# gyroflow/gyroflow

Measured on NVIDIA H100. Metric: 4K frames/sec (fisheye+RS warp), higher is better.
Workload: dtype f32

## Files before the change

### gyroflow_b200/csrc/c_abi.cu

```cuda
#include <cuda_runtime.h>
#include <cstdio>
#include <cstring>
#include <cstdlib>
#include <mutex>
#include <cmath>
#include <algorithm>
#include <string>
#include <vector>

#include "kernel_registry.h"
#include "c_abi_internal.h"
#include "gyro_dev.h"
#include <nvtx3/nvToolsExt.h>

using namespace gf;

namespace {

struct Slot {
    GrowBuf<float, true> h_mat, h_mesh;
    GrowBuf<float> d_mat, d_mesh;
    GrowBuf<double> d_mesh64;
    Event done;
};
constexpr int kSlots = 4;
constexpr int kPackedBlockY = 4;
constexpr unsigned long long kMaxOutRows = 65535ull * GF_BLOCK_Y;
static_assert(2 * kPackedBlockY == GF_BLOCK_Y, "the packed kernel's row blocks cover GF_BLOCK_Y rows, like the scalar kernels'");

struct LayoutInfo { int bpp, channels, scalar; float max_value; };
constexpr LayoutInfo kLayouts[LAY_COUNT] = {
    { 1, 1, SC_U8,  255.0f },          { 2, 2, SC_U8,  255.0f },          { 3, 3, SC_U8,  255.0f },   { 4, 4, SC_U8,  255.0f },
    { 2, 1, SC_U16, 65535.0f },        { 4, 2, SC_U16, 65535.0f },        { 6, 3, SC_U16, 65535.0f }, { 8, 4, SC_U16, 65535.0f },
    { 4, 1, SC_F32, 3.402823466e38f }, { 16, 4, SC_F32, 3.402823466e38f }, { 8, 4, SC_F16, 3.402823466e38f },
};

struct Combo {
    int lens = 0, digital = 0, layout = 0;
    KernelFn kernels[KV_COUNT] = {};
    bool no_filter = false;
    int bpp() const { return kLayouts[layout].bpp; }
};

}

struct gf_cuda_ctx {
    int device = 0;
    Combo combo;
    int interpolation = 0;
    int width = 0, height = 0, output_width = 0, output_height = 0;
    KernelFn fn_shade = nullptr;
    GrowBuf<uint32_t> const_flags;
    GrowBuf<uint32_t> vflags;
    cudaStream_t last_stream = nullptr;
    Event last_call;
    FilterPrepass filter;
    int overlays = 0;
    GrowBuf<uint8_t, true> h_drawing;
    GrowBuf<uint8_t> d_drawing, src_ovl;
    PlaneStaging plane_staging;
    size_t host_in_len = 0, host_out_len = 0;
    GrowBuf<uint2> coords;
    Stream stream;
    size_t max_rows = 0;
    Slot slots[kSlots];
    int next_slot = 0;
    unsigned long long launches = 0;
    std::string last_error;
};

namespace {

int pix_layout(int pixel_type) {
    static constexpr int kPixLayout[GF_PIX_COUNT] = { LAY_1U8, LAY_1U16, LAY_3U8, LAY_4U8, LAY_4U8, LAY_3U16, LAY_4U16, LAY_4U16,
                                                      LAY_4F32, LAY_4F16, LAY_1F32, LAY_2U8, LAY_2U16 };
    return (pixel_type >= 0 && pixel_type < GF_PIX_COUNT) ? kPixLayout[pixel_type] : -1;
}

KernelFn find_kernel(const Combo& c, int interp, KernelVariant v) {
    switch (c.lens) {
    case GF_LENS_OPENCV_FISHEYE:     return gf_kernel_opencv_fisheye(c.digital, c.layout, interp, v);
    case GF_LENS_OPENCV_STANDARD:    return gf_kernel_opencv_standard(c.digital, c.layout, interp, v);
    case GF_LENS_POLY3:              return gf_kernel_poly3(c.digital, c.layout, interp, v);
    case GF_LENS_POLY5:              return gf_kernel_poly5(c.digital, c.layout, interp, v);
    case GF_LENS_PTLENS:             return gf_kernel_ptlens(c.digital, c.layout, interp, v);
    case GF_LENS_INSTA360:           return gf_kernel_insta360(c.digital, c.layout, interp, v);
    case GF_LENS_SONY:               return gf_kernel_sony(c.digital, c.layout, interp, v);
    case GF_LENS_GENERIC_POLYNOMIAL: return gf_kernel_generic_polynomial(c.digital, c.layout, interp, v);
    case GF_LENS_GOPRO:              return gf_kernel_gopro(c.digital, c.layout, interp, v);
    default: return nullptr;
    }
}

bool make_combo(int pixel_type, int lens, int digital, int interp, Combo* c) {
    c->layout = pix_layout(pixel_type); c->lens = lens; c->digital = digital;
    const bool no_lean = getenv("GF_DISABLE_LEAN") != nullptr;
    const bool no_packed = no_lean || getenv("GF_DISABLE_X2") != nullptr;
    c->no_filter = getenv("GF_DISABLE_FILTER") != nullptr;
    for (int v = 0; v < KV_COUNT; ++v)
        c->kernels[v] = ((no_packed && v >= KV_PACKED) || (no_lean && v == KV_LEAN)) ? nullptr : find_kernel(*c, interp, (KernelVariant)v);
    return c->layout >= 0;
}

const char* const kLensNames[GF_LENS_COUNT] = {
    "none", "opencv_fisheye", "opencv_standard", "poly3", "poly5", "ptlens", "insta360", "sony", "generic_polynomial",
    "gopro", "gopro_superview", "gopro_hyperview", "gopro_warp", "digital_stretch", "gopro6_superview" };

int validate(std::string* err, const gf_kernel_params* p, const gf_buffer_desc* in, const gf_buffer_desc* out, int bpp) {
    if (!p || !in || !out) return fail(err, GF_ERR_BAD_PARAMS, "null argument");
    if (in->height < 4 || out->height < 4 || p->height < 4 || p->output_height < 4)
        return fail(err, GF_ERR_SIZE_TOO_SMALL, "SizeTooSmall: height < 4");
    if (p->stride < 1 || p->output_stride < 1) return fail(err, GF_ERR_BAD_STRIDE, "InvalidStride: stride < 1");
    if (p->width > 16384 || p->output_width > 16384 || p->width < 1 || p->output_width < 1)
        return fail(err, GF_ERR_BAD_PARAMS, "width out of range (1..16384)");
    if (in->width > p->stride)         return fail(err, GF_ERR_BAD_STRIDE, "InvalidStride: input width > stride");
    if (out->width > p->output_stride) return fail(err, GF_ERR_BAD_STRIDE, "InvalidStride: output width > output_stride");
    if (p->stride != in->stride || p->output_stride != out->stride)
        return fail(err, GF_ERR_BAD_STRIDE, "InvalidStride: KernelParams stride differs from the buffer description");
    if (p->bytes_per_pixel != bpp) return fail(err, GF_ERR_BAD_PARAMS, "bytes_per_pixel does not match the pixel type");
    if (p->matrix_count < 1) return fail(err, GF_ERR_BAD_PARAMS, "matrix_count < 1");
    if ((in->kind != GF_BUF_HOST && in->kind != GF_BUF_DEVICE) || (out->kind != GF_BUF_HOST && out->kind != GF_BUF_DEVICE) || !in->ptr || !out->ptr)
        return fail(err, GF_ERR_BAD_PARAMS, "unsupported buffer source");
    const long long x0 = p->source_rect[0], y0 = p->source_rect[1], x1 = x0 + p->source_rect[2], y1 = y0 + p->source_rect[3];
    if (p->source_rect[2] > 0 && p->source_rect[3] > 0) {
        if (x0 < 0 || y0 < 0) return fail(err, GF_ERR_BUFFER_TOO_SMALL, "source_rect has a negative origin");
        const unsigned long long last = (unsigned long long)(y1 - 1) * (unsigned long long)p->stride + (unsigned long long)x1 * (unsigned long long)bpp;
        if (last > in->len) return fail(err, GF_ERR_BUFFER_TOO_SMALL, "Buffer size mismatch input: source_rect exceeds the input buffer");
    }
    if (out->len == 0) return fail(err, GF_ERR_BUFFER_TOO_SMALL, "empty output buffer");
    const unsigned long long out_rows = (out->len + (unsigned long long)p->output_stride - 1) / (unsigned long long)p->output_stride;
    if (p->output_stride < bpp || out_rows > kMaxOutRows)
        return fail(err, GF_ERR_BAD_PARAMS, "output buffer geometry out of range (a pixel per row, at most 524280 rows)");
    return GF_OK;
}

__global__ void widen_mesh_kernel(const float* __restrict__ m, double* __restrict__ o, int n, float width_f, float height_f) {
    const int i = blockIdx.x * blockDim.x + threadIdx.x;
    if (i < n) o[i] = (double)m[i];
    if (i == 0 && n >= 9) make_mesh_aux(m, width_f, height_f, *reinterpret_cast<MeshAux*>(o + GF_MESH_MAX_LEN));
}
__global__ void __launch_bounds__(1024) scan_tables_kernel(const float* __restrict__ m, size_t rows, uint32_t* flags) {
    __shared__ unsigned warp_or[32];
    unsigned f = 0;
    const size_t n = rows * GF_MATRIX_STRIDE;
    for (size_t i = threadIdx.x; i < n; i += blockDim.x) f |= table_entry_verdict((unsigned)(i % GF_MATRIX_STRIDE), m[i]);
    f = __reduce_or_sync(0xffffffffu, f);
    if ((threadIdx.x & 31u) == 0u) warp_or[threadIdx.x >> 5] = f;
    __syncthreads();
    if (threadIdx.x < 32u) {
        f = threadIdx.x < (blockDim.x >> 5) ? warp_or[threadIdx.x] : 0u;
        f = __reduce_or_sync(0xffffffffu, f);
        if (threadIdx.x == 0u) *flags = f;
    }
}

void fill_uniforms(WarpArgs& A, const Combo& c) {
    const gf_kernel_params* p = &A.p;
    const uint8_t* const src = A.src;
    const uint8_t* const dst = A.dst;
    const int bpp = c.bpp();
    A.out_rows = (int)((A.dst_len + (size_t)p->output_stride - 1) / (size_t)p->output_stride);
    A.out_cols = p->output_stride / bpp;
    const int align = (bpp == 1 || bpp == 2 || bpp == 4 || bpp == 8 || bpp == 16) ? bpp : (bpp == 3 ? 1 : 2);
    uint32_t f = 0;
    if (p->matrix_count > 1) f |= F_RS;
    if ((p->flags & 16) == 16) f |= F_HRS;
    A.r_limit_sq = p->r_limit * p->r_limit;
    if (A.r_limit_sq > 0.0f) f |= F_RLIMIT;
    if (p->light_refraction_coefficient != 1.0f && p->light_refraction_coefficient > 0.0f) f |= F_REFRACT;
    if (A.mesh_len > 0) f |= F_MESH;
    if ((p->flags & 2) == 2 && c.digital != GF_LENS_NONE) f |= F_DIGITAL;
    if (p->input_horizontal_stretch > 0.001f && p->input_horizontal_stretch != 1.0f) f |= F_HSTRETCH;
    if (p->input_vertical_stretch   > 0.001f && p->input_vertical_stretch   != 1.0f) f |= F_VSTRETCH;
    if (p->lens_correction_amount < 1.0f) f |= F_LCA;
    if (p->input_rotation != 0.0f) f |= F_INROT;
    if (p->background_mode == 1) f |= F_BG1;
    if (p->background_mode == 2) f |= F_BG2;
    if (p->background_mode == 3) f |= F_BG3;
    if ((p->flags & 1) == 1) f |= F_FIXRANGE;
    if ((p->flags & 4) == 4) f |= F_FILLBG;
    if (lens_noop(c.lens, p->k)) f |= F_LENS_NOOP;
// ... 154 lines not shown
        }
        if (job.tables_on_device) {
            T.table_flags = job.table_flags_dev ? job.table_flags_dev : ctx->const_flags.ptr + 1;
            T.matrices = job.matrices;
            T.mesh = job.mesh_len ? job.mesh : nullptr;
        } else {
            for (size_t i = 0; i < job.n; ++i) table_rows = std::max(table_rows, (size_t)p[i].matrix_count);
            const size_t mat_bytes = table_rows * GF_MATRIX_STRIDE * sizeof(float);
            memcpy(slot->h_mat.ptr, job.matrices, mat_bytes);
            table_flags = gf_table_flags_host(slot->h_mat.ptr, table_rows);
            CK(err, cudaMemcpyAsync(slot->d_mat.ptr, slot->h_mat.ptr, mat_bytes, cudaMemcpyHostToDevice, st));
            T.matrices = slot->d_mat.ptr;
            if (job.mesh_len) {
                memcpy(slot->h_mesh.ptr, job.mesh, job.mesh_len * sizeof(float));
                CK(err, cudaMemcpyAsync(slot->d_mesh.ptr, slot->h_mesh.ptr, job.mesh_len * sizeof(float), cudaMemcpyHostToDevice, st));
                T.mesh = slot->d_mesh.ptr;
            }
        }
        T.mesh_len = (int)job.mesh_len;
        if (job.mesh_len) {
            double* const m64 = slot->d_mesh64.ptr;
            widen_mesh_kernel<<<(unsigned)((job.mesh_len + 255) / 256), 256, 0, st>>>(T.mesh, m64, (int)job.mesh_len, (float)p->width, (float)p->height);
            CK(err, cudaGetLastError());
            T.mesh64 = m64; T.mesh_aux = reinterpret_cast<const MeshAux*>(m64 + GF_MESH_MAX_LEN);
        }
        if (host) {
            nvtxRangePushA("gf_h2d_frame");
            const int rc = ctx->plane_staging.upload(job.n, job.in, job.out, p, false, st, err, in.data(), out.data());
            nvtxRangePop();
            if (rc != GF_OK) return rc;
            src_private = job.in[0].kind == GF_BUF_HOST;
        }
        return GF_OK;
    }

    int draw_input_overlays() {
        if (!overlays || job.n != 1) return GF_OK;
        bool any_input_stage = false;
        if ((p->flags & GF_FLAG_DRAWING_ENABLED) && job.drawing && job.drawing_len) {
            CK(err, ctx->h_drawing.reserve(job.drawing_len, st));
            CK(err, ctx->d_drawing.reserve(job.drawing_len, st));
            CK(err, cudaStreamSynchronize(st));
            for (size_t i = 0; i < job.drawing_len; ++i) { const uint8_t d = job.drawing[i]; ctx->h_drawing.ptr[i] = d; any_input_stage |= (d != 0 && (d & 1u) == 0u); }
            CK(err, cudaMemcpyAsync(ctx->d_drawing.ptr, ctx->h_drawing.ptr, job.drawing_len, cudaMemcpyHostToDevice, st));
            drawing_dev = ctx->d_drawing.ptr;
        }
        if (!any_input_stage) return GF_OK;
        if (!src_private) {
            CK(err, ctx->src_ovl.reserve(in[0].len, st));
            CK(err, cudaMemcpyAsync(ctx->src_ovl.ptr, in[0].ptr, in[0].len, cudaMemcpyDeviceToDevice, st));
            in[0].ptr = ctx->src_ovl.ptr;
        }
        const LayoutInfo& L = kLayouts[ctx->combo.layout];
        if (gf_internal_draw_overlays((void*)st, (uint8_t*)in[0].ptr, in[0].len, in[0].width, in[0].height, p->stride, p, L.channels, L.scalar, 1,
                                      drawing_dev, job.drawing_len) != GF_OK) return fail(err, GF_ERR_CUDA, "overlay kernel (input stage) failed");
        return GF_OK;
    }

    int render() {
        if (fused) return render_planes(0, job.n);
        for (size_t i = 0; i < job.n; ++i) { const int rc = render_planes(i, 1); if (rc != GF_OK) return rc; }
        return GF_OK;
    }

    int render_planes(size_t first, size_t count) {
        WarpArgs A = T;
        A.p = p[first];
        A.src = (const uint8_t*)in[first].ptr; A.dst = (uint8_t*)out[first].ptr; A.src_len = in[first].len; A.dst_len = out[first].len;
        const uint32_t flags = (size_t)A.p.matrix_count < table_rows ? gf_table_flags_host(slot->h_mat.ptr, (size_t)A.p.matrix_count) : table_flags;
        if (!job.tables_on_device) A.table_flags = ctx->const_flags.ptr + (flags ? 1 : 0);
        fill_uniforms(A, ctx->combo);
        const dim3 grid((A.out_cols + GF_BLOCK_X - 1) / GF_BLOCK_X, (A.out_rows + GF_BLOCK_Y - 1) / GF_BLOCK_Y);
        const Plan plan = plan_frame(ctx->combo, A, flags, job.tables_on_device, count, job.coord_only);
        const FilterPrepass::Table* radial = nullptr;
        if (plan.filter) { const int rc = ctx->filter.table(A.p.k, st, err, &radial); if (rc != GF_OK) return rc; }
        if (plan.two_pass) {
            if (!ctx->fn_shade && !job.coord_only) return fail(err, GF_ERR_UNSUPPORTED_COMBO, "no sampling kernel for this pixel layout");
            CK(err, ctx->coords.reserve((size_t)A.out_cols * (size_t)A.out_rows * (size_t)plan.n_maps, st));
            A.coord_out = ctx->coords.ptr;
        }
        const KernelFn fn = ctx->combo.kernels[plan.kernel];
        if (plan.kernel == KV_PACKED || plan.kernel == KV_PACKED_COORDS) {
            const dim3 block2(GF_BLOCK_X, kPackedBlockY), grid2(grid.x, (A.out_rows + 2 * kPackedBlockY - 1) / (2 * kPackedBlockY));
            if (radial) { const int rc = ctx->filter.launch(fn, grid2, block2, A, *radial, st, err, ctx->launches); if (rc != GF_OK) return rc; }
            else CK(err, launch_pdl(fn, grid2, block2, A, st));
        } else {
            const size_t map_len = (size_t)A.out_cols * (size_t)A.out_rows;
            for (int mi = 0; mi < plan.n_maps; ++mi) {
                if (plan.two_pass) { A.coord_out = ctx->coords.ptr + (size_t)mi * map_len; A.coord_shift = mi; }
                fn<<<grid, kBlock, 0, st>>>(A);
                CK(err, cudaGetLastError());
                if (mi > 0) ctx->launches++;
            }
        }
        CK(err, cudaGetLastError());
        ctx->launches++;
        if (!plan.two_pass || job.coord_only) return GF_OK;
        for (size_t i = first; i < first + count; ++i) {
            WarpArgs B = A;
            B.p = p[i];
            B.coord_out = nullptr; B.coord_in = ctx->coords.ptr; B.coord_maps = plan.n_maps; B.coord_shift = 0;
            B.src = (const uint8_t*)in[i].ptr; B.dst = (uint8_t*)out[i].ptr; B.src_len = in[i].len; B.dst_len = out[i].len;
            fill_uniforms(B, ctx->combo);
            ctx->fn_shade<<<grid, kBlock, 0, st>>>(B);
            CK(err, cudaGetLastError());
            ctx->launches++;
        }
        return GF_OK;
    }

    int finish() {
        if (slot) CK(err, cudaEventRecord(slot->done.get(), st));
        for (size_t i = 0; overlays && i < job.n; ++i) {
            const LayoutInfo& L = kLayouts[ctx->combo.layout];
            if (gf_internal_draw_overlays((void*)st, (uint8_t*)out[i].ptr, out[i].len, out[i].width, out[i].height, p[i].output_stride, &p[i], L.channels,
                                          L.scalar, 0, drawing_dev, job.drawing_len) != GF_OK) return fail(err, GF_ERR_CUDA, "overlay kernel (output stage) failed");
        }
        if (!host) return GF_OK;
        nvtxRangePushA("gf_d2h_frame");
        const int rc = ctx->plane_staging.download(job.n, job.out, p, st, err);
        nvtxRangePop();
        if (rc != GF_OK) return rc;
        if (job.sync_host) CK(err, cudaStreamSynchronize(st));
        return GF_OK;
    }
};

int order_after_last_call(gf_cuda_ctx* ctx, cudaStream_t st) {
    if (ctx->last_stream && ctx->last_stream != st) CK(&ctx->last_error, cudaStreamWaitEvent(st, ctx->last_call.get(), 0));
    ctx->last_stream = st;
    return GF_OK;
}

int check_frame(gf_cuda_ctx* ctx, const FrameJob& job) {
    std::string* const err = &ctx->last_error;
    for (size_t i = 0; i < job.n; ++i) {
        if (job.kind >= 0 && (job.in[i].kind != job.kind || job.out[i].kind != job.kind)) return fail(err, GF_ERR_BAD_PARAMS, job.kind_error);
        const int rc = validate(err, job.p + i, job.in + i, job.out + i, ctx->combo.bpp());
        if (rc != GF_OK) return rc;
    }
    for (size_t i = 0; i < job.n; ++i) {
        const gf_kernel_params* p = &job.p[i];
        if (!job.matrices) return fail(err, GF_ERR_NO_DATA, "NoStabilizationData: matrices is null");
        if (p->width != ctx->width || p->height != ctx->height || p->output_width != ctx->output_width || p->output_height != ctx->output_height)
            return fail(err, GF_ERR_SIZE_MISMATCH, "SizeMismatch: KernelParams size differs from the size this context was created for");
        if (p->interpolation != ctx->interpolation)
            return fail(err, GF_ERR_UNSUPPORTED_COMBO, "interpolation differs from the one this context was created for");
        if ((size_t)p->matrix_count > job.matrix_rows) return fail(err, GF_ERR_BUFFER_TOO_SMALL, "Buffer size mismatch matrices: matrix_count > rows supplied");
        if (!job.tables_on_device && job.matrix_rows > ctx->max_rows) return fail(err, GF_ERR_BUFFER_TOO_SMALL, "Buffer size mismatch matrices");
        if (job.mesh_len > GF_MESH_MAX_LEN) return fail(err, GF_ERR_BUFFER_TOO_SMALL, "Buffer size mismatch buf_mesh_data");
        if (job.mesh_len > 0 && !job.mesh) return fail(err, GF_ERR_BAD_PARAMS, "mesh is null");
        if (job.mesh_len > 0 && job.mesh_len < 9) return fail(err, GF_ERR_BAD_PARAMS, "mesh shorter than its 9-value header (the reference would index out of bounds)");
        if (!job.grow_staging && job.in[i].kind == GF_BUF_HOST && job.in[i].len > ctx->host_in_len)
            return fail(err, GF_ERR_BUFFER_TOO_SMALL, "Buffer size mismatch input");
        if (!job.grow_staging && job.out[i].kind == GF_BUF_HOST && job.out[i].len > ctx->host_out_len)
            return fail(err, GF_ERR_BUFFER_TOO_SMALL, "Buffer size mismatch output");
        if (job.tables_on_device && (reinterpret_cast<uintptr_t>(job.matrices) & 7u)) return fail(err, GF_ERR_BAD_PARAMS, "device matrices must be 8-byte aligned");
    }
    return GF_OK;
}

int run_frame(gf_cuda_ctx* ctx, const FrameJob& job) {
    if (!ctx) return fail(nullptr, GF_ERR_BAD_PARAMS, "ctx is null");
    std::string* const err = &ctx->last_error;
    int rc = check_frame(ctx, job);
    if (rc != GF_OK) return rc;
    CK(err, cudaSetDevice(ctx->device));
// ... 461 lines not shown
```

### gyroflow_b200/csrc/c_abi_internal.h

```cpp
#pragma once
#include <cuda_runtime.h>
#include <cstddef>
#include <cstdint>
#include <memory>
#include <string>
#include <vector>
#include "../../include/gyroflow_cuda.h"
#include "frame_geometry.cuh"

namespace gf {


inline thread_local std::string g_last_error;

inline int fail(std::string* sink, int code, const std::string& msg) {
    g_last_error = msg;
    if (sink) *sink = msg;
    return code;
}
inline int cuda_error(cudaError_t e, const char* what, std::string* sink) {
    (void)cudaGetLastError();
    return fail(sink, GF_ERR_CUDA, std::string(what) + ": " + cudaGetErrorName(e) + " (" + cudaGetErrorString(e) + ")");
}
#define CK(sink, call) do { const cudaError_t e_ = (call); if (e_ != cudaSuccess) return gf::cuda_error(e_, #call, sink); } while (0)


template <class T, bool PINNED = false> struct GrowBuf {
    T* ptr = nullptr; size_t len = 0;
    GrowBuf() = default;
    GrowBuf(GrowBuf&& o) noexcept : ptr(o.ptr), len(o.len) { o.ptr = nullptr; o.len = 0; }
    ~GrowBuf() { release(); }
    cudaError_t reserve(size_t n, cudaStream_t st) {
        if (n <= len) return cudaSuccess;
        if (ptr) { const cudaError_t e = cudaStreamSynchronize(st); if (e != cudaSuccess) return e; release(); }
        const cudaError_t e = PINNED ? cudaMallocHost((void**)&ptr, n * sizeof(T)) : cudaMalloc((void**)&ptr, n * sizeof(T));
        if (e == cudaSuccess) len = n; else ptr = nullptr;
        return e;
    }
private:
    void release() { if (ptr) { if (PINNED) cudaFreeHost(ptr); else cudaFree(ptr); } ptr = nullptr; len = 0; }
};

template <auto Destroy> struct Deleter { template <class T> void operator()(T* h) const { Destroy(h); } };
using Stream = std::unique_ptr<CUstream_st, Deleter<cudaStreamDestroy>>;
using Event = std::unique_ptr<CUevent_st, Deleter<cudaEventDestroy>>;
inline cudaError_t create_stream(Stream& s) {
    cudaStream_t h = nullptr;
    const cudaError_t e = cudaStreamCreateWithFlags(&h, cudaStreamNonBlocking);
    if (e == cudaSuccess) s.reset(h);
    return e;
}
inline cudaError_t create_event(Event& ev) {
    cudaEvent_t h = nullptr;
    const cudaError_t e = cudaEventCreateWithFlags(&h, cudaEventDisableTiming);
    if (e == cudaSuccess) ev.reset(h);
    return e;
}

enum : uint32_t { TBL_WILD = 1u, TBL_IBIS = 2u };
__host__ __device__ __forceinline__ bool tame(float v) { const float a = fabsf(v); return v == 0.0f || (a >= 0x1p-40f && a <= 0x1p40f); }
__host__ __device__ __forceinline__ uint32_t table_entry_verdict(unsigned col, float v) {
    return col < 9u ? (tame(v) ? 0u : TBL_WILD) : (v == 0.0f ? 0u : TBL_IBIS);
}
__host__ __device__ __forceinline__ uint32_t table_row_verdict(const float* r) {
    uint32_t f = 0;
    for (unsigned i = 0; i < GF_MATRIX_STRIDE; ++i) f |= table_entry_verdict(i, r[i]);
    return f;
}

double keyframed(const gf_compute_params* cp, int typ, double timestamp_ms, double dflt);
double fov_unscaled(const gf_compute_params* cp, size_t frame, bool use_fovs, double timestamp_ms, bool for_ui);
void get_new_k(const gf_compute_params* cp, const double* camera_matrix, double fov, double (&new_k)[9]);
struct FrameTiming {
    double frame_readout_time;
    double row_readout_time, start_ts;
    Quat q0;
};
FrameTiming frame_timing(const gf_compute_params* cp, size_t frame, double timestamp_ms, bool can_invert);
CameraStab camera_stab_at(const gf_compute_params* cp, size_t frame, bool framebuffer_inverted, const StabSplines* splines);
bool lens_noop(int lens, const float* k);
bool point_path_supported(int lens, int digital);

struct WarpArgs;
typedef void (*KernelFn)(const WarpArgs);
cudaError_t launch_pdl(KernelFn fn, dim3 g, dim3 b, const WarpArgs& args, cudaStream_t st);
float radial_table_cap(const float* k, float4* rows);
class FilterPrepass {
public:
    struct Table {
        uint32_t key[4] = {};
        float a_cap = 0.0f;
        unsigned long long last_use = 0;
        GrowBuf<float4, true> h; GrowBuf<float4> d; Event done;
    };
    cudaError_t init(int device) { return cudaDeviceGetAttribute(&sm_count, cudaDevAttrMultiProcessorCount, device); }
    int table(const float* k, cudaStream_t st, std::string* err, const Table** out);
    int launch(KernelFn fn, dim3 grid, dim3 block, WarpArgs& A, const Table& t, cudaStream_t st, std::string* err, unsigned long long& launches);
    int stats(cudaStream_t st, std::string* err, uint64_t* out6) const;
private:
    Table tables[4];
    GrowBuf<uint32_t> queue; GrowBuf<unsigned> counts;
    unsigned long long frames = 0, uses = 0, builds = 0;
    int sm_count = 1;
};

bool warp_covers_output(const gf_kernel_params& p, const gf_buffer_desc& out, int bpp);
class PlaneStaging {
public:
    cudaError_t reserve(size_t n, const gf_buffer_desc* in, const gf_buffer_desc* out, cudaStream_t st);
    int check(size_t n, const gf_buffer_desc* in, const gf_buffer_desc* out, std::string* err) const;
    int upload(size_t n, const gf_buffer_desc* in, const gf_buffer_desc* out, const gf_kernel_params* p, bool checksum, cudaStream_t st,
               std::string* err, gf_buffer_desc* din, gf_buffer_desc* dout);
    int download(size_t n, const gf_buffer_desc* out, const gf_kernel_params* p, cudaStream_t st, std::string* err) const;
private:
    std::vector<GrowBuf<uint8_t>> in_, out_;
};

inline gf_compute_params stmap_params(const gf_compute_params& user, int per_frame) {
    gf_compute_params cp = user;
    if (!per_frame) cp.frame_readout_time = 0.0;
    cp.suppress_rotation = 1; cp.fovs = nullptr; cp.n_fovs = 0; cp.minimal_fovs = nullptr; cp.n_minimal_fovs = 0;
    cp.fov_scale = 1.0; cp.output_width = cp.width; cp.output_height = cp.height;
    return cp;
}
inline bool stmap_size_ok(int w, int h) { return w >= 4 && h >= 4 && w <= 32768 && h <= 32768; }

}

int gf_internal_draw_overlays(void* cu_stream, uint8_t* buf_dev, size_t len, int width, int height, int stride, const gf_kernel_params* p,
                              int count, int scalar, int is_input, const uint8_t* drawing_dev, size_t drawing_len);
```

### gyroflow_b200/csrc/filter_prepass.cu

```cuda
#include <cstring>
#include <cmath>
#include <algorithm>
#include "warp_kernel.cuh"
#include "c_abi_internal.h"

using namespace gf;
namespace {

constexpr unsigned kDeferCap = 1u << 20;
constexpr unsigned kTailThreadsPerSM = 2048;

float filter_a_cap(const float* k) {
    auto B = [&](double t) { const double t2 = t * t; return t2 * (fabs((double)k[0]) + t2 * (fabs((double)k[1]) + t2 * (fabs((double)k[2]) + t2 * fabs((double)k[3])))); };
    for (int i = 0; i < 4; ++i) if (!std::isfinite(k[i])) return 0.0f;
    double lo = 0.0, hi = 1.55;
    if (B(hi) > 0.25) { for (int it = 0; it < 60; ++it) { const double mid = 0.5 * (lo + hi); if (B(mid) <= 0.25) lo = mid; else hi = mid; } }
    else lo = hi;
    if (lo < 0.5) return 0.0f;
    const double a = tan(lo) * tan(lo);
    return (float)std::min(a * 0.999, 16000.0);
}

double radial_T(double a) { const double r = sqrt(a); return r < 1e-4 ? 1.0 - a / 3.0 + a * a / 5.0 : atan(r) / r; }
struct RadialGrid {
    static constexpr int N = GF_RADIAL_FIT_ROWS, kChk = 65;
    double lo[N], hi[N], h[N];
    double node_a[N][4], node_T[N][4];
    double chk_a[N][kChk], chk_T[N][kChk];
    double vinv[4][4];
    RadialGrid() {
        double t[4], V[4][8];
        for (int q = 0; q < 4; ++q) t[q] = cos((2 * q + 1) * 3.14159265358979323846 / 8.0);
        for (int r = 0; r < 4; ++r) for (int c = 0; c < 8; ++c) V[r][c] = c < 4 ? pow(1.0 + t[r], c) : (c - 4 == r ? 1.0 : 0.0);
        for (int c = 0; c < 4; ++c) {
            int p = c;
            for (int r = c + 1; r < 4; ++r) if (fabs(V[r][c]) > fabs(V[p][c])) p = r;
            for (int j = 0; j < 8; ++j) std::swap(V[c][j], V[p][j]);
            const double d = V[c][c];
            for (int j = 0; j < 8; ++j) V[c][j] /= d;
            for (int r = 0; r < 4; ++r) if (r != c) { const double f = V[r][c]; for (int j = 0; j < 8; ++j) V[r][j] -= f * V[c][j]; }
        }
        for (int r = 0; r < 4; ++r) for (int c = 0; c < 4; ++c) vinv[r][c] = V[r][c + 4];
        for (int i = 0; i < N; ++i) {
            const int e = i / 16, j = i % 16;
            lo[i] = ldexp(1.0 + j / 16.0, e - 30); hi[i] = ldexp(1.0 + (j + 1) / 16.0, e - 30);
            h[i] = 0.5 * (hi[i] - lo[i]);
            for (int q = 0; q < 4; ++q) { node_a[i][q] = lo[i] + h[i] * (1.0 + t[q]); node_T[i][q] = radial_T(node_a[i][q]); }
            for (int q = 0; q < kChk; ++q) { chk_a[i][q] = (double)(float)(lo[i] + (hi[i] - lo[i]) * q / 64.0); chk_T[i][q] = radial_T(chk_a[i][q]); }
        }
    }
};

float build_radial_table(const float* k, float a_cap, float4* rows) {
    static const RadialGrid* const G = new RadialGrid();
    constexpr double kRadialBudget = 0x1p-23;
    uint32_t cap_bits; memcpy(&cap_bits, &a_cap, 4);
    const int n_valid = std::max(0, std::min(GF_RADIAL_FIT_ROWS, (int)(cap_bits >> 19) - GF_RADIAL_FIT));
    const double k0 = k[0], k1 = k[1], k2 = k[2], k3 = k[3];
    auto R = [&](double a, double T) { const double q = a * T * T; return T * (1.0 + q * (k0 + q * (k1 + q * (k2 + q * k3)))); };
    bool ok = n_valid > 0;
    for (int i = 0; i < GF_RADIAL_ROWS; ++i) rows[i] = make_float4(NAN, NAN, NAN, NAN);
    for (int i = 0; i < n_valid; ++i) {
        double f[4], c[4];
        for (int q = 0; q < 4; ++q) f[q] = R(G->node_a[i][q], G->node_T[i][q]);
        for (int r = 0; r < 4; ++r) c[r] = G->vinv[r][0] * f[0] + G->vinv[r][1] * f[1] + G->vinv[r][2] * f[2] + G->vinv[r][3] * f[3];
        const double hh = G->h[i];
        const float4 row = make_float4((float)c[0], (float)(c[1] / hh), (float)(c[2] / (hh * hh)), (float)(c[3] / (hh * hh * hh)));
        rows[GF_RADIAL_FIT + i] = row;
        for (int q = 0; q < RadialGrid::kChk; ++q) {
            const double a = G->chk_a[i][q], d = a - G->lo[i];
            const double v = row.x + d * (row.y + d * (row.z + d * (double)row.w));
            const double want = R(a, G->chk_T[i][q]);
            if (!(fabs(v - want) <= kRadialBudget * fabs(want))) ok = false;
        }
    }
    for (int i = 0; i < GF_RADIAL_FIT; ++i) rows[i] = rows[GF_RADIAL_FIT];
    uint32_t r_bits = cap_bits & 0xfff80000u; float a_cap_r; memcpy(&a_cap_r, &r_bits, 4);
    return ok ? a_cap_r : 0.0f;
}

}

float gf::radial_table_cap(const float* k, float4* rows) { return build_radial_table(k, filter_a_cap(k), rows); }

int FilterPrepass::table(const float* k, cudaStream_t st, std::string* err, const Table** out) {
    uint32_t key[4]; memcpy(key, k, sizeof(key));
    Table *t = nullptr, *lru = &tables[0];
    for (Table& e : tables) {
        if (e.last_use && memcmp(e.key, key, sizeof(key)) == 0) t = &e;
        if (e.last_use < lru->last_use) lru = &e;
    }
    if (!t) {
        t = lru; t->last_use = 0;
        if (!t->done) CK(err, create_event(t->done));
        CK(err, cudaEventSynchronize(t->done.get()));
        CK(err, t->h.reserve(GF_RADIAL_ROWS, st)); CK(err, t->d.reserve(GF_RADIAL_ROWS, st));
        t->a_cap = radial_table_cap(k, t->h.ptr); builds++;
        CK(err, cudaMemcpyAsync(t->d.ptr, t->h.ptr, GF_RADIAL_ROWS * sizeof(float4), cudaMemcpyHostToDevice, st));
        CK(err, cudaEventRecord(t->done.get(), st));
        memcpy(t->key, key, sizeof(key));
    }
    t->last_use = ++uses;
    *out = t->a_cap > 0.0f ? t : nullptr;
    return GF_OK;
}

int FilterPrepass::launch(KernelFn fn, dim3 grid, dim3 block, WarpArgs& A, const Table& t, cudaStream_t st, std::string* err,
                          unsigned long long& launches) {
    if (!queue.ptr) {
        CK(err, queue.reserve(kDeferCap, st)); CK(err, counts.reserve(2, st));
        CK(err, cudaMemsetAsync(counts.ptr, 0, 2 * sizeof(unsigned), st));
    }
    const unsigned cur = (unsigned)(frames++ & 1ull);
    A.feat |= F_FILTER;
    A.flt.q = queue.ptr; A.flt.cap = (uint32_t)queue.len;
    A.flt.count = counts.ptr + cur; A.flt.count_next = counts.ptr + (cur ^ 1u);
    A.flt.mid_row = A.matrices + (size_t)(A.p.matrix_count / 2) * GF_MATRIX_STRIDE;
    const FilterEps eps = filter_eps(A.p.c[1]);
    A.flt.rtab = t.d.ptr; A.flt.eps_rel = eps.rel; A.flt.eps_abs = eps.abs;
    A.flt.tail = 0;
    CK(err, launch_pdl(fn, grid, block, A, st));
    CK(err, cudaEventRecord(t.done.get(), st));
    A.flt.tail = 1;
    CK(err, launch_pdl(fn, dim3(sm_count * kTailThreadsPerSM / (block.x * block.y)), block, A, st));
    launches++;
    return GF_OK;
}

int FilterPrepass::stats(cudaStream_t st, std::string* err, uint64_t* out6) const {
    unsigned count = 0;
    if (frames > 0) {
        CK(err, cudaMemcpyAsync(&count, counts.ptr + ((frames - 1) & 1ull), sizeof(count), cudaMemcpyDeviceToHost, st));
        CK(err, cudaStreamSynchronize(st));
    }
    out6[0] = frames; out6[1] = count; out6[2] = kDeferCap; out6[3] = (uint64_t)sm_count * kTailThreadsPerSM;
    out6[4] = builds; out6[5] = uses - builds;
    return GF_OK;
}
```

### gyroflow_b200/csrc/warp_kernel.cuh

```cuda
#pragma once
#include "lens_models.cuh"
#include "gf_coeffs_tables.h"
#include "f32x2.cuh"
#include <cuda_fp16.h>

namespace gf {

struct MapC {
    float in_min, mul, div, rcp, add;
    int   fast_div;
    int   identity;
};

__host__ __device__ inline MapC make_map(float in_min, float in_max, float out_min, float out_max, float max_abs_int_coord) {
    MapC m;
    m.in_min = in_min;
    m.mul = out_max - out_min;
    m.div = in_max - in_min;
    m.rcp = 1.0f / m.div;
    m.add = out_min;
    const float ad = fabsf(m.div);
    m.fast_div = (isfinite(m.div) && ad >= 0x1p-40f && ad <= 0x1p40f) ? 1 : 0;
    m.identity = (max_abs_int_coord >= 0.0f && m.mul == m.div && m.mul > 0.0f && in_min == truncf(in_min) &&
                  (max_abs_int_coord + fabsf(in_min)) * m.mul < 16777216.0f) ? 1 : 0;
    return m;
}

enum : uint32_t {
    F_RS         = 1u << 0,
    F_HRS        = 1u << 1,
    F_RLIMIT     = 1u << 2,
    F_REFRACT    = 1u << 3,
    F_MESH       = 1u << 4,
    F_DIGITAL    = 1u << 5,
    F_HSTRETCH   = 1u << 6,
    F_VSTRETCH   = 1u << 7,
    F_LCA        = 1u << 8,
    F_INROT      = 1u << 9,
    F_BG1        = 1u << 10,
    F_BG2        = 1u << 11,
    F_BG3        = 1u << 12,
    F_FIXRANGE   = 1u << 13,
    F_FILLBG     = 1u << 14,
    F_LENS_NOOP  = 1u << 15,
    F_SRC_VEC    = 1u << 16,
    F_DST_VEC    = 1u << 17,
    F_FB_INV     = 1u << 18,
    F_IS_Y       = 1u << 19,
    F_T3D        = 1u << 20,
    F_PIXLIMIT   = 1u << 21,
    F_WILD       = 1u << 22,
    F_INTPRO     = 1u << 23,
    F_FILTER     = 1u << 24,
    F_SRC_VEC8   = 1u << 25,
    F_SHORTROW   = 1u << 26,
};

constexpr uint32_t F_GENERAL_ONLY = F_HRS | F_RLIMIT | F_REFRACT | F_MESH | F_HSTRETCH | F_VSTRETCH | F_LCA | F_INROT |
                                    F_BG1 | F_BG2 | F_BG3 | F_FIXRANGE | F_FILLBG | F_LENS_NOOP | F_FB_INV | F_T3D | F_PIXLIMIT;
constexpr uint32_t F_LEAN_REQUIRED = F_SRC_VEC | F_DST_VEC;

template <bool GEN> __device__ __forceinline__ bool has(uint32_t feat, uint32_t bit) {
    if (GEN) return (feat & bit) != 0;
    if (bit & F_GENERAL_ONLY) return false;
    if (bit & (F_LEAN_REQUIRED | F_DIGITAL)) return true;
    return (feat & bit) != 0;
}

constexpr int GF_RADIAL_ROWS = 8192;
constexpr int GF_RADIAL_FIT = (127 - 30) << 4;
constexpr int GF_RADIAL_FIT_ROWS = (14 + 30) * 16;

constexpr float kFilterRho = 0x1.7p-18f;
struct FilterEps { float rel, abs; };
GF_HD FilterEps filter_eps(float c_y, float rho = kFilterRho) { return { rho + 0x1p-22f, 0x1p-22f * fabsf(c_y) }; }

struct WarpArgs {
    gf_kernel_params p;
    const uint8_t* src;
    uint8_t*       dst;
    const float*   matrices;
    const float*   mesh;
    const double*  mesh64;
    const struct MeshAux* mesh_aux;
    uint2*         coord_out;
    const uint2*   coord_in;
    const uint32_t* table_flags;
    struct X2Filter {
        static constexpr int kMaxCols = 1 << 16, kMaxRows = 2 << 16;
        uint32_t* q;
        unsigned* count;
        unsigned* count_next;
        uint32_t  cap;
        int       tail;
        const float4* rtab;
        const float*  mid_row;
        float     eps_rel, eps_abs;
    } flt;
    int            coord_shift;
    int            coord_maps;
    unsigned long long src_len, dst_len;
    int   mesh_len;
    int   out_rows;
    int   out_cols;
    uint32_t feat;
    float r_limit_sq;
    float out_c[2], out_f[2];
    float bg[4];
    MapC  omap_x, omap_y;
    MapC  smap_x, smap_y;
    float width_f, height_f;
    float frame_w, frame_h;
    float rot_cos, rot_sin;
    int   rs_lim;
    int   row_lim;
    int   u8_limit;
    int   src_rect[4];
    int   interior_span[2];
    struct X2Hot {
        const uint8_t* src;
        int x_off, y_off;
        int x0, x1, y0, y1;
        int full_rows, last_cols;
        int wbias[2];
        unsigned wlim[2];
        int full;
    } hot;
};

enum { SC_U8 = 0, SC_U16 = 1, SC_F32 = 2, SC_F16 = 3 };

template <int COUNT_, int SCALAR_> struct Pix {
    static constexpr int COUNT = COUNT_;
    static constexpr int SCALAR = SCALAR_;
    static constexpr int SBYTES = SCALAR_ == SC_U8 ? 1 : (SCALAR_ == SC_F32 ? 4 : 2);
    static constexpr int BYTES = COUNT_ * SBYTES;
    static constexpr bool POW2 = (BYTES == 1 || BYTES == 2 || BYTES == 4 || BYTES == 8 || BYTES == 16);
    static constexpr int ALIGN = POW2 ? BYTES : SBYTES;

    static GF_DEV float scalar_to_float(uint32_t raw) {
        if (SCALAR == SC_F32) return __uint_as_float(raw);
        if (SCALAR == SC_F16) return __half2float(__ushort_as_half((unsigned short)raw));
        return __uint_as_float(0x4b000000u | raw) - 8388608.0f;
    }
    static GF_DEV uint32_t float_to_scalar(float v) {
        if (SCALAR == SC_F32) return __float_as_uint(v);
        if (SCALAR == SC_F16) {
            const uint32_t b = __float_as_uint(v);
            if (v != v) return ((b >> 16) & 0x8000u) | 0x7e00u | ((b & 0x7fffffu) >> 13);
            return (uint32_t)__half_as_ushort(__float2half_rn(v));
        }
        int i = __float2int_rz(v);
        const int hi = SCALAR == SC_U8 ? 255 : 65535;
        i = i < 0 ? 0 : (i > hi ? hi : i);
        return (uint32_t)i;
    }
    static GF_DEV uint32_t load_scalar(const uint8_t* __restrict__ p) {
        if (SBYTES == 1) return __ldg(p);
        if (SBYTES == 2) return __ldg(reinterpret_cast<const unsigned short*>(p));
        return __ldg(reinterpret_cast<const unsigned int*>(p));
    }
    static GF_DEV void load_raw(const uint8_t* __restrict__ p, uint32_t (&r)[COUNT]) {
        if (!POW2) {
            #pragma unroll
            for (int i = 0; i < COUNT; ++i) r[i] = load_scalar(p + i * SBYTES);
        } else if (BYTES <= 4) {
            const uint32_t w = BYTES == 1 ? (uint32_t)__ldg(p) : (BYTES == 2 ? (uint32_t)__ldg(reinterpret_cast<const unsigned short*>(p)) : __ldg(reinterpret_cast<const unsigned int*>(p)));
            #pragma unroll
            for (int i = 0; i < COUNT; ++i) r[i] = COUNT == 1 ? w : ((w >> (8 * SBYTES * i)) & (SBYTES == 1 ? 0xffu : 0xffffu));
        } else if (BYTES == 8) {
            const uint2 w = __ldg(reinterpret_cast<const uint2*>(p));
            #pragma unroll
// ... 922 lines not shown
```

### gyroflow_b200/csrc/warp_kernel_x2.cuh

```cuda
#pragma once
#include "warp_kernel.cuh"

namespace gf {

using p2::f2;

GF_DEV bool in_window_r2(float a) {
    const uint32_t t = (__float_as_uint(a) << 1) - (71u << 24);
    return t < (104u << 24);
}
GF_DEV bool zero_or_in_window(float v) {
    const uint32_t u = __float_as_uint(v) << 1;
    return u == 0u || (u - (67u << 24)) < (121u << 24);
}

template <int M> struct Lens2 { static constexpr bool kHas = false; };
__host__ __device__ constexpr bool filter_pair(int lens, int digital) { return lens == GF_LENS_OPENCV_FISHEYE && digital == GF_LENS_NONE; }

template <> struct Lens2<GF_LENS_OPENCV_FISHEYE> {
    static constexpr bool kHas = true;
    static GF_DEV bool divisors_ok(float wa, float wb) { return fminf(wa, wb) > 0.0f; }
    static GF_DEV float approx_v(float _x, float _y, float _w, const gf_kernel_params& P, const float4* __restrict__ rtab) {
        const float iw = p2::rcp_approx(_w);
        const float x = _x * iw, y = _y * iw;
// ... 487 lines not shown
template <int LENS, int DIGITAL, class PIX, bool COORD>
static __device__ __noinline__ void finish_pair_cold(const WarpArgs& A, int x, int y0, float pxs, f2 py, uint32_t idx_a, uint32_t idx_b,
                                                     bool wr_a, bool wr_b) {
    const PairUV c = rotate_and_distort_cold<LENS, DIGITAL>(pxs, py.x, py.y, idx_a, idx_b, A, 1);
    const bool ok_a = (c.ok & 1) != 0, ok_b = (c.ok & 2) != 0;
    if (COORD) {
        uint2* const cm_a = A.coord_out + ((size_t)y0 * (size_t)A.out_cols + (size_t)x);
        *cm_a = !wr_a ? make_uint2(GF_COORD_MARK, GF_COORD_SKIP) : (ok_a ? make_uint2(__float_as_uint(c.ua), __float_as_uint(c.va)) : make_uint2(GF_COORD_MARK, GF_COORD_NONE));
        if ((y0 + 1) < A.out_rows) cm_a[A.out_cols] = !wr_b ? make_uint2(GF_COORD_MARK, GF_COORD_SKIP) : (ok_b ? make_uint2(__float_as_uint(c.ub), __float_as_uint(c.vb)) : make_uint2(GF_COORD_MARK, GF_COORD_NONE));
        return;
    }
    const unsigned long long off_a = (unsigned long long)y0 * (unsigned long long)A.p.output_stride + (unsigned long long)x * (unsigned long long)PIX::BYTES;
    int wu_a = 0, wu_b = 0, wv_a = 0, wv_b = 0;
    if (PIX::SCALAR == SC_U8) {
        wu_a = hot_w(c.ua, A.hot.wbias[0]); wv_a = hot_w(c.va, A.hot.wbias[1]);
        wu_b = hot_w(c.ub, A.hot.wbias[0]); wv_b = hot_w(c.vb, A.hot.wbias[1]);
    }
    if (wr_a) shade_lean<PIX>(ok_a, (c.ok & 4) != 0, c.ua, c.va, wu_a, wv_a, A, A.dst + off_a);
    if (wr_b) shade_lean<PIX>(ok_b, (c.ok & 8) != 0, c.ub, c.vb, wu_b, wv_b, A, A.dst + off_a + (unsigned long long)A.p.output_stride);
}

template <int LENS, int DIGITAL, class PIX, bool TRUSTED, bool COORD, bool FULL = false>
GF_DEV void warp_x2_body(const WarpArgs& A, const int x, const int y0, const bool exact_prepass) {
    using namespace p2;
    static_assert(!FULL || DIGITAL == GF_LENS_NONE, "a digital lens may turn a coordinate into -0");
    const gf_kernel_params& P = A.p;
    if (!FULL && (x >= A.out_cols || y0 >= A.out_rows)) return;
    const unsigned long long BYTES = COORD ? (unsigned long long)P.bytes_per_pixel : (unsigned long long)PIX::BYTES;
    const unsigned long long ostride = (unsigned long long)P.output_stride;
    const unsigned long long off_a = (unsigned long long)y0 * ostride + (unsigned long long)x * BYTES;
    const unsigned long long off_b = off_a + ostride;
    float opx, opy_a, opy_b;
    bool wr_a, wr_b;
    if (FULL) {
        wr_a = wr_b = true;
        opx = (float)(x + A.hot.x_off); opy_a = (float)(y0 + A.hot.y_off); opy_b = (float)(y0 + 1 + A.hot.y_off);
    } else if (A.feat & F_INTPRO) {
        const int y1 = y0 + 1;
        const bool in_x = (x >= A.hot.x0) & (x < A.hot.x1);
        wr_a = in_x & (y0 >= A.hot.y0) & (y0 < A.hot.y1);
        wr_b = in_x & (y1 >= A.hot.y0) & (y1 < A.hot.y1);
        if (A.feat & F_SHORTROW) {
            wr_a &= (y0 < A.hot.full_rows) | ((y0 == A.hot.full_rows) & (x < A.hot.last_cols));
            wr_b &= (y1 < A.hot.full_rows) | ((y1 == A.hot.full_rows) & (x < A.hot.last_cols));
        }
        opx = (float)(x + A.hot.x_off); opy_a = (float)(y0 + A.hot.y_off); opy_b = (float)(y1 + A.hot.y_off);
    } else {
        opx = map_apply_int_lean((float)x, A.omap_x);
        opy_a = map_apply_int_lean((float)y0, A.omap_y);
        opy_b = map_apply_int_lean((float)(y0 + 1), A.omap_y);
        const bool in_x = (opx >= 0.0f) & (as_i32(opx) < P.output_width);
        wr_a = in_x & (off_a + BYTES <= A.dst_len) & (opy_a >= 0.0f) & (as_i32(opy_a) < P.output_height);
        wr_b = in_x & ((y0 + 1) < A.out_rows) & (off_b + BYTES <= A.dst_len) & (opy_b >= 0.0f) & (as_i32(opy_b) < P.output_height);
    }
    uint2* const cm_a = COORD ? A.coord_out + ((size_t)y0 * (size_t)A.out_cols + (size_t)x) : nullptr;
    const bool row_b = FULL || (y0 + 1) < A.out_rows;
    if (!FULL && !(wr_a | wr_b)) {
        if (COORD) { *cm_a = make_uint2(GF_COORD_MARK, GF_COORD_SKIP); if (row_b) cm_a[A.out_cols] = make_uint2(GF_COORD_MARK, GF_COORD_SKIP); }
        return;
    }

    const float pxs = opx + P.translation2d[0];
    const f2 px = bc(pxs);
    const f2 py = mk(opy_a + P.translation2d[1], opy_b + P.translation2d[1]);
    const int lim = A.row_lim;
    int sy_a = 0, sy_b = 0;
    do {
        if constexpr (TRUSTED && filter_pair(LENS, DIGITAL)) {
            if (!exact_prepass) {
                const MatRow9 rm = load_row9(A.flt.mid_row, 0u);
                const float bx = pxs * rm.m01.x, by = pxs * rm.m23.y, bw = pxs * rm.m67.x;
                const float xa = (bx + py.x * rm.m01.y) + rm.m23.x, xb = (bx + py.y * rm.m01.y) + rm.m23.x;
                const float ya = (by + py.x * rm.m45.x) + rm.m45.y, yb = (by + py.y * rm.m45.x) + rm.m45.y;
                const float wa = (bw + py.x * rm.m67.y) + rm.m8,    wb = (bw + py.y * rm.m67.y) + rm.m8;
                const float ca = Lens2<LENS>::approx_v(xa, ya, wa, P, A.flt.rtab), cb = Lens2<LENS>::approx_v(xb, yb, wb, P, A.flt.rtab);
                const bool w_ok = Lens2<LENS>::divisors_ok(wa, wb);
                const float ta = ca + P.c[1], tb = cb + P.c[1];
                const float ea = __fmaf_rn(fabsf(ca), A.flt.eps_rel, A.flt.eps_abs), eb = __fmaf_rn(fabsf(cb), A.flt.eps_rel, A.flt.eps_abs);
                const bool ca_ok = certify_row(ta, ea, lim, sy_a), cb_ok = certify_row(tb, eb, lim, sy_b);
                if (w_ok & ca_ok & cb_ok) break;
                const unsigned m = __activemask();
                const unsigned lane = threadIdx.x & 31u;
                const int leader = __ffs((int)m) - 1;
                unsigned base = 0;
                if ((int)lane == leader) base = atomicAdd(A.flt.count, (unsigned)__popc(m));
                base = __shfl_sync(m, base, leader);
                const unsigned slot = base + (unsigned)__popc(m & ((1u << lane) - 1u));
                if (slot < A.flt.cap) { A.flt.q[slot] = (uint32_t)x | ((uint32_t)(y0 >> 1) << 16); return; }
            } else if (!(A.feat & F_RS)) break;
        } else {
            if (!(A.feat & F_RS)) break;
        }
        const uint32_t mid = (uint32_t)P.matrix_count / 2u;
        f2 tu, tv; bool bad = false;
        rotate_and_distort_x2<LENS, DIGITAL, TRUSTED>(px, py, mid, mid, A, tu, tv, bad);
        if (bad) {
            const PairUV c = rotate_and_distort_cold<LENS, DIGITAL>(pxs, py.x, py.y, mid, mid, A, 0);
            tv = mk((c.ok & 1) ? c.va : py.x, (c.ok & 2) ? c.vb : py.y);
        }
        round_away_clamped_x2(tv, lim, sy_a, sy_b);
    } while (false);
    f2 u, v; bool bad = false;
    rotate_and_distort_x2<LENS, DIGITAL, TRUSTED>(px, py, (uint32_t)sy_a, (uint32_t)sy_b, A, u, v, bad);
    u = map_apply_x2<!FULL>(u, A.smap_x, bad);
    v = map_apply_x2<!FULL>(v, A.smap_y, bad);
    if (bad) { finish_pair_cold<LENS, DIGITAL, PIX, COORD>(A, x, y0, pxs, py, (uint32_t)sy_a, (uint32_t)sy_b, wr_a, wr_b); return; }

    if (COORD) {
        *cm_a = !wr_a ? make_uint2(GF_COORD_MARK, GF_COORD_SKIP) : make_uint2(__float_as_uint(u.x), __float_as_uint(v.x));
        if (row_b) cm_a[A.out_cols] = !wr_b ? make_uint2(GF_COORD_MARK, GF_COORD_SKIP) : make_uint2(__float_as_uint(u.y), __float_as_uint(v.y));
        return;
    }
    int wu_a = 0, wu_b = 0, wv_a = 0, wv_b = 0;
    if (PIX::SCALAR == SC_U8) {
        wu_a = hot_w(u.x, A.hot.wbias[0]); wv_a = hot_w(v.x, A.hot.wbias[1]);
        wu_b = hot_w(u.y, A.hot.wbias[0]); wv_b = hot_w(v.y, A.hot.wbias[1]);
        if (wr_a & wr_b & hot_interior(wu_a, wv_a, A) & hot_interior(wu_b, wv_b, A)) {
            constexpr int C = PIX::COUNT;
            uint32_t sa[C], sb[C];
            sample_u8_hot<PIX>(wu_a, wv_a, A, sa);
            sample_u8_hot<PIX>(wu_b, wv_b, A, sb);
            PIX::store_scalars(A.dst + off_a, true, sa);
            PIX::store_scalars(A.dst + off_b, true, sb);
            return;
        }
    }
    if (wr_a) shade_lean<PIX>(true, false, u.x, v.x, wu_a, wv_a, A, A.dst + off_a);
    if (wr_b) shade_lean<PIX>(true, false, u.y, v.y, wu_b, wv_b, A, A.dst + off_b);
}

template <int LENS, int DIGITAL, class PIX, int MINB, bool COORD = false>
__global__ void __launch_bounds__(GF_BLOCK_X * GF_BLOCK_Y, MINB)
warp_kernel_x2(const __grid_constant__ WarpArgs A) {
    constexpr bool kFilter = filter_pair(LENS, DIGITAL);
    asm volatile("griddepcontrol.wait;" ::: "memory");
    const bool trusted = __ldg(A.table_flags) == 0u;
    if constexpr (kFilter) if (A.flt.tail) {
        const unsigned tid = (blockIdx.y * gridDim.x + blockIdx.x) * (blockDim.x * blockDim.y) + threadIdx.y * blockDim.x + threadIdx.x;
        if (tid == 0u) *A.flt.count_next = 0u;
        if (!trusted) return;
        const unsigned n = min(*A.flt.count, A.flt.cap);
        const unsigned stride = gridDim.x * gridDim.y * blockDim.x * blockDim.y;
        for (unsigned i = tid; i < n; i += stride) {
            const uint32_t e = A.flt.q[i];
            warp_x2_body<LENS, DIGITAL, PIX, true, COORD>(A, (int)(e & 0xffffu), (int)(e >> 16) * 2, true);
        }
        return;
    }
    const int x = blockIdx.x * GF_BLOCK_X + threadIdx.x;
    const int y0 = (blockIdx.y * blockDim.y + threadIdx.y) * 2;
    if (trusted) {
        const bool exact_prepass = !(kFilter && (A.feat & F_FILTER));
        if constexpr (DIGITAL == GF_LENS_NONE) if (A.hot.full) { warp_x2_body<LENS, DIGITAL, PIX, true, COORD, true>(A, x, y0, exact_prepass); return; }
        warp_x2_body<LENS, DIGITAL, PIX, true, COORD>(A, x, y0, exact_prepass);
    } else {
        warp_x2_body<LENS, DIGITAL, PIX, false, COORD>(A, x, y0, true);
    }
}

}
```

Before: 11190.

## Shard filter defer-queue counter into padded segments to cut atomic contention

Replaces the single global atomic counter for the deferred-pixel queue with 128 padded per-segment counters and sub-queues, selected by warp row index, so warps enqueueing failed-certification pixels contend less on one address. The tail pass now assigns warps to segments and strides within each segment, and stats sum all segment counts. It also adds an env-controlled epsilon scale for the filter tolerance, which defaults to 1 and so changes nothing by default. The cost is that per-segment capacity is cap/128, so a skewed segment can overflow sooner, and the tail work may be unevenly balanced across segments.

Result: no change. 11240 (median of 6 runs) (+0.5%).

```diff
diff --git a/gyroflow_b200/csrc/c_abi.cu b/gyroflow_b200/csrc/c_abi.cu
--- a/gyroflow_b200/csrc/c_abi.cu
+++ b/gyroflow_b200/csrc/c_abi.cu
@@ -39,6 +39,7 @@
     int lens = 0, digital = 0, layout = 0;
     KernelFn kernels[KV_COUNT] = {};
     bool no_filter = false;
+    float eps_scale = 1.0f;
     int bpp() const { return kLayouts[layout].bpp; }
 };
 
@@ -97,6 +98,7 @@
     const bool no_lean = getenv("GF_DISABLE_LEAN") != nullptr;
     const bool no_packed = no_lean || getenv("GF_DISABLE_X2") != nullptr;
     c->no_filter = getenv("GF_DISABLE_FILTER") != nullptr;
+    if (const char* e = getenv("GF_FILTER_EPS_SCALE")) { const float v = strtof(e, nullptr); if (v >= 1.0f) c->eps_scale = v; }
     for (int v = 0; v < KV_COUNT; ++v)
         c->kernels[v] = ((no_packed && v >= KV_PACKED) || (no_lean && v == KV_LEAN)) ? nullptr : find_kernel(*c, interp, (KernelVariant)v);
     return c->layout >= 0;
@@ -417,7 +419,7 @@
         const KernelFn fn = ctx->combo.kernels[plan.kernel];
         if (plan.kernel == KV_PACKED || plan.kernel == KV_PACKED_COORDS) {
             const dim3 block2(GF_BLOCK_X, kPackedBlockY), grid2(grid.x, (A.out_rows + 2 * kPackedBlockY - 1) / (2 * kPackedBlockY));
-            if (radial) { const int rc = ctx->filter.launch(fn, grid2, block2, A, *radial, st, err, ctx->launches); if (rc != GF_OK) return rc; }
+            if (radial) { const int rc = ctx->filter.launch(fn, grid2, block2, A, *radial, ctx->combo.eps_scale, st, err, ctx->launches); if (rc != GF_OK) return rc; }
             else CK(err, launch_pdl(fn, grid2, block2, A, st));
         } else {
             const size_t map_len = (size_t)A.out_cols * (size_t)A.out_rows;
diff --git a/gyroflow_b200/csrc/c_abi_internal.h b/gyroflow_b200/csrc/c_abi_internal.h
--- a/gyroflow_b200/csrc/c_abi_internal.h
+++ b/gyroflow_b200/csrc/c_abi_internal.h
@@ -95,7 +95,8 @@
     };
     cudaError_t init(int device) { return cudaDeviceGetAttribute(&sm_count, cudaDevAttrMultiProcessorCount, device); }
     int table(const float* k, cudaStream_t st, std::string* err, const Table** out);
-    int launch(KernelFn fn, dim3 grid, dim3 block, WarpArgs& A, const Table& t, cudaStream_t st, std::string* err, unsigned long long& launches);
+    int launch(KernelFn fn, dim3 grid, dim3 block, WarpArgs& A, const Table& t, float eps_scale, cudaStream_t st, std::string* err,
+               unsigned long long& launches);
     int stats(cudaStream_t st, std::string* err, uint64_t* out6) const;
 private:
     Table tables[4];
diff --git a/gyroflow_b200/csrc/filter_prepass.cu b/gyroflow_b200/csrc/filter_prepass.cu
--- a/gyroflow_b200/csrc/filter_prepass.cu
+++ b/gyroflow_b200/csrc/filter_prepass.cu
@@ -1,6 +1,7 @@
 #include <cstring>
 #include <cmath>
 #include <algorithm>
+#include <vector>
 #include "warp_kernel.cuh"
 #include "c_abi_internal.h"
 
@@ -9,6 +10,7 @@
 
 constexpr unsigned kDeferCap = 1u << 20;
 constexpr unsigned kTailThreadsPerSM = 2048;
+constexpr unsigned kCounts = 2 * WarpArgs::X2Filter::kSegs * WarpArgs::X2Filter::kCountStride;
 
 float filter_a_cap(const float* k) {
     auto B = [&](double t) { const double t2 = t * t; return t2 * (fabs((double)k[0]) + t2 * (fabs((double)k[1]) + t2 * (fabs((double)k[2]) + t2 * fabs((double)k[3])))); };
@@ -105,19 +107,19 @@
     return GF_OK;
 }
 
-int FilterPrepass::launch(KernelFn fn, dim3 grid, dim3 block, WarpArgs& A, const Table& t, cudaStream_t st, std::string* err,
-                          unsigned long long& launches) {
+int FilterPrepass::launch(KernelFn fn, dim3 grid, dim3 block, WarpArgs& A, const Table& t, float eps_scale, cudaStream_t st,
+                          std::string* err, unsigned long long& launches) {
     if (!queue.ptr) {
-        CK(err, queue.reserve(kDeferCap, st)); CK(err, counts.reserve(2, st));
-        CK(err, cudaMemsetAsync(counts.ptr, 0, 2 * sizeof(unsigned), st));
+        CK(err, queue.reserve(kDeferCap, st)); CK(err, counts.reserve(kCounts, st));
+        CK(err, cudaMemsetAsync(counts.ptr, 0, kCounts * sizeof(unsigned), st));
     }
     const unsigned cur = (unsigned)(frames++ & 1ull);
     A.feat |= F_FILTER;
-    A.flt.q = queue.ptr; A.flt.cap = (uint32_t)queue.len;
-    A.flt.count = counts.ptr + cur; A.flt.count_next = counts.ptr + (cur ^ 1u);
+    A.flt.q = queue.ptr; A.flt.cap = (uint32_t)(queue.len / WarpArgs::X2Filter::kSegs);
+    A.flt.count = counts.ptr + cur * (kCounts / 2); A.flt.count_next = counts.ptr + (cur ^ 1u) * (kCounts / 2);
     A.flt.mid_row = A.matrices + (size_t)(A.p.matrix_count / 2) * GF_MATRIX_STRIDE;
     const FilterEps eps = filter_eps(A.p.c[1]);
-    A.flt.rtab = t.d.ptr; A.flt.eps_rel = eps.rel; A.flt.eps_abs = eps.abs;
+    A.flt.rtab = t.d.ptr; A.flt.eps_rel = eps.rel * eps_scale; A.flt.eps_abs = eps.abs * eps_scale;
     A.flt.tail = 0;
     CK(err, launch_pdl(fn, grid, block, A, st));
     CK(err, cudaEventRecord(t.done.get(), st));
@@ -128,10 +130,12 @@
 }
 
 int FilterPrepass::stats(cudaStream_t st, std::string* err, uint64_t* out6) const {
-    unsigned count = 0;
+    uint64_t count = 0;
     if (frames > 0) {
-        CK(err, cudaMemcpyAsync(&count, counts.ptr + ((frames - 1) & 1ull), sizeof(count), cudaMemcpyDeviceToHost, st));
+        std::vector<unsigned> c(kCounts / 2);
+        CK(err, cudaMemcpyAsync(c.data(), counts.ptr + ((frames - 1) & 1ull) * (kCounts / 2), c.size() * sizeof(unsigned), cudaMemcpyDeviceToHost, st));
         CK(err, cudaStreamSynchronize(st));
+        for (unsigned s = 0; s < WarpArgs::X2Filter::kSegs; ++s) count += c[s * WarpArgs::X2Filter::kCountStride];
     }
     out6[0] = frames; out6[1] = count; out6[2] = kDeferCap; out6[3] = (uint64_t)sm_count * kTailThreadsPerSM;
     out6[4] = builds; out6[5] = uses - builds;
diff --git a/gyroflow_b200/csrc/warp_kernel.cuh b/gyroflow_b200/csrc/warp_kernel.cuh
--- a/gyroflow_b200/csrc/warp_kernel.cuh
+++ b/gyroflow_b200/csrc/warp_kernel.cuh
@@ -88,6 +88,7 @@
     const uint32_t* table_flags;
     struct X2Filter {
         static constexpr int kMaxCols = 1 << 16, kMaxRows = 2 << 16;
+        static constexpr unsigned kSegs = 128, kCountStride = 32;
         uint32_t* q;
         unsigned* count;
         unsigned* count_next;
diff --git a/gyroflow_b200/csrc/warp_kernel_x2.cuh b/gyroflow_b200/csrc/warp_kernel_x2.cuh
--- a/gyroflow_b200/csrc/warp_kernel_x2.cuh
+++ b/gyroflow_b200/csrc/warp_kernel_x2.cuh
@@ -593,11 +593,12 @@
                 const unsigned m = __activemask();
                 const unsigned lane = threadIdx.x & 31u;
                 const int leader = __ffs((int)m) - 1;
+                const unsigned seg = ((blockIdx.y * gridDim.x + blockIdx.x) * blockDim.y + threadIdx.y) % WarpArgs::X2Filter::kSegs;
                 unsigned base = 0;
-                if ((int)lane == leader) base = atomicAdd(A.flt.count, (unsigned)__popc(m));
+                if ((int)lane == leader) base = atomicAdd(A.flt.count + seg * WarpArgs::X2Filter::kCountStride, (unsigned)__popc(m));
                 base = __shfl_sync(m, base, leader);
                 const unsigned slot = base + (unsigned)__popc(m & ((1u << lane) - 1u));
-                if (slot < A.flt.cap) { A.flt.q[slot] = (uint32_t)x | ((uint32_t)(y0 >> 1) << 16); return; }
+                if (slot < A.flt.cap) { A.flt.q[seg * A.flt.cap + slot] = (uint32_t)x | ((uint32_t)(y0 >> 1) << 16); return; }
             } else if (!(A.feat & F_RS)) break;
         } else {
             if (!(A.feat & F_RS)) break;
@@ -648,12 +649,15 @@
     const bool trusted = __ldg(A.table_flags) == 0u;
     if constexpr (kFilter) if (A.flt.tail) {
         const unsigned tid = (blockIdx.y * gridDim.x + blockIdx.x) * (blockDim.x * blockDim.y) + threadIdx.y * blockDim.x + threadIdx.x;
-        if (tid == 0u) *A.flt.count_next = 0u;
+        constexpr unsigned S = WarpArgs::X2Filter::kSegs;
+        if (tid < S) A.flt.count_next[tid * WarpArgs::X2Filter::kCountStride] = 0u;
         if (!trusted) return;
-        const unsigned n = min(*A.flt.count, A.flt.cap);
-        const unsigned stride = gridDim.x * gridDim.y * blockDim.x * blockDim.y;
-        for (unsigned i = tid; i < n; i += stride) {
-            const uint32_t e = A.flt.q[i];
+        const unsigned warp = tid >> 5, seg = warp % S;
+        const unsigned n = min(A.flt.count[seg * WarpArgs::X2Filter::kCountStride], A.flt.cap);
+        const unsigned per_seg = gridDim.x * gridDim.y * blockDim.x * blockDim.y / 32u / S;
+        const unsigned i0 = warp / S < per_seg ? (warp / S) * 32u + (tid & 31u) : n;
+        for (unsigned i = i0; i < n; i += per_seg * 32u) {
+            const uint32_t e = A.flt.q[seg * A.flt.cap + i];
             warp_x2_body<LENS, DIGITAL, PIX, true, COORD>(A, (int)(e & 0xffffu), (int)(e >> 16) * 2, true);
         }
         return;
```
